# nagadomi/nunif

Hardware: NVIDIA H100
Metric: waifu2x_input_megapixels_per_sec (higher is better)
Workload: dtype f16

## Files before the change

nunif_b200/csrc/gemm.cu:

```cuda
#include "gemm.h"
#include "gemm_wgmma.cuh"
#include "tmap.h"
#include "../../include/nunif_b200.h"
#include <mutex>
#include <cstdlib>

namespace nb200 {

typedef CUresult (*EncodeTiledFn)(CUtensorMap*, CUtensorMapDataType, cuuint32_t, void*, const cuuint64_t*,
                                  const cuuint64_t*, const cuuint32_t*, const cuuint32_t*, CUtensorMapInterleave,
                                  CUtensorMapSwizzle, CUtensorMapL2promotion, CUtensorMapFloatOOBfill);

static EncodeTiledFn get_encode() {
    static EncodeTiledFn fn = nullptr;
    static std::once_flag once;
    std::call_once(once, [] {
        void* p = nullptr;
        cudaDriverEntryPointQueryResult q;
        if (cudaGetDriverEntryPoint("cuTensorMapEncodeTiled", &p, cudaEnableDefault, &q) == cudaSuccess &&
            q == cudaDriverEntryPointSuccess)
            fn = (EncodeTiledFn)p;
    });
    return fn;
}

int encode(CUtensorMap* m, const void* base, int rank, const cuuint64_t* dims, const cuuint64_t* strides_bytes,
                  const cuuint32_t* box, int swizzle_bytes) {
    EncodeTiledFn fn = get_encode();
    if (!fn) return fail("cuTensorMapEncodeTiled is not available (no CUDA driver?)");
    cuuint32_t estr[5] = {1, 1, 1, 1, 1};
    CUtensorMapSwizzle sw = swizzle_bytes == 128 ? CU_TENSOR_MAP_SWIZZLE_128B
                                                 : (swizzle_bytes == 64 ? CU_TENSOR_MAP_SWIZZLE_64B : CU_TENSOR_MAP_SWIZZLE_32B);
    CUresult r = fn(m, CU_TENSOR_MAP_DATA_TYPE_FLOAT16, (cuuint32_t)rank, const_cast<void*>(base), dims, strides_bytes, box,
                    estr, CU_TENSOR_MAP_INTERLEAVE_NONE, sw, CU_TENSOR_MAP_L2_PROMOTION_L2_256B,
                    CU_TENSOR_MAP_FLOAT_OOB_FILL_NONE);
    if (r != CUDA_SUCCESS) return fail("cuTensorMapEncodeTiled failed with CUresult " + std::to_string((int)r));
    return 0;
}

template <int BN, int BK, bool A2 = false>
static int launch_t(cudaStream_t st, const GemmMaps& maps, const GemmParams& p, int m_tiles, int n_tiles) {
    using Cfg = GemmCfg<BN, BK>;
    if (ensure_dyn_smem((const void*)gemm_conv_kernel<BN, BK, A2>, Cfg::SMEM_BYTES)) return 1;
    cudaLaunchConfig_t cfg = {};
    cfg.gridDim = dim3((unsigned)m_tiles * n_tiles); cfg.blockDim = dim3(GEMM_THREADS); cfg.dynamicSmemBytes = Cfg::SMEM_BYTES;
    cfg.stream = st;
    cudaLaunchAttribute at[1];
    at[0].id = cudaLaunchAttributeProgrammaticStreamSerialization;
    at[0].val.programmaticStreamSerializationAllowed = 1;
    cfg.attrs = at; cfg.numAttrs = 1;
    NB_CUDA(cudaLaunchKernelEx(&cfg, gemm_conv_kernel<BN, BK, A2>, maps, p));
    NB_LAUNCHED();
    return 0;
}

template <int BK>
static int launch_bn(int bn, cudaStream_t st, const GemmMaps& maps, const GemmParams& p, int m_tiles, int n_tiles) {
    if (p.k2) switch (bn) {
        case 64: return launch_t<64, BK, true>(st, maps, p, m_tiles, n_tiles);
        case 96: return launch_t<96, BK, true>(st, maps, p, m_tiles, n_tiles);
        default: return fail("second A operand: unsupported BLOCK_N");
    }
    switch (bn) {
        case 16: return launch_t<16, BK>(st, maps, p, m_tiles, n_tiles);
        case 32: return launch_t<32, BK>(st, maps, p, m_tiles, n_tiles);
        case 48: return launch_t<48, BK>(st, maps, p, m_tiles, n_tiles);
        case 64: return launch_t<64, BK>(st, maps, p, m_tiles, n_tiles);
        case 96: return launch_t<96, BK>(st, maps, p, m_tiles, n_tiles);
        case 128: return launch_t<128, BK>(st, maps, p, m_tiles, n_tiles);
    }
    return fail("unsupported BLOCK_N");
}

static int num_sms() { return device_sm_count(); }

std::atomic<int> g_tune_epoch{0};
int g_tune[16] = {0, 0, 0,  0, 0, 0,  0,
                   0, 0,  0, 0, 0, 0, 0, 0, 0};

static int encode_nhwc4(CUtensorMap* m, const __half* base, int C, int X, int Y, int B, long long sx, long long sy, long long sb,
                        int cw, int tw, int th) {
    cuuint64_t dims[4] = {(cuuint64_t)C, (cuuint64_t)X, (cuuint64_t)Y, (cuuint64_t)B};
    cuuint64_t strides[3] = {(cuuint64_t)sx * 2, (cuuint64_t)sy * 2, (cuuint64_t)sb * 2};
    cuuint32_t box[4] = {(cuuint32_t)cw, (cuuint32_t)tw, (cuuint32_t)th, 1};
    return encode(m, base, 4, dims, strides, box, cw * 2);
}

int conv_gemm(cudaStream_t st, const ConvGemm& g) {
    NB_CHECK(g.A && g.Wt && g.out, "null pointer");
    NB_CHECK(g.Ci % 8 == 0, "input channel stride must be a multiple of 8");
    NB_CHECK(g.N % 16 == 0, "N must be a multiple of 16 (pad the weights)");
    GemmParams p;
    memset(&p, 0, sizeof(p));
    int ktap;
    cuuint64_t dims[5], strides[4];
    cuuint32_t box[5];
    const cuuint64_t e = 2;
    const cuuint64_t rs = (g.a_row_stride ? (cuuint64_t)g.a_row_stride : (cuuint64_t)g.Wi * g.Ci) * e;
    const cuuint64_t is = (g.a_img_stride ? (cuuint64_t)g.a_img_stride * e : (cuuint64_t)g.Hi * rs);
    switch (g.kind) {
        case CG_LINEAR_FLAT: {
            const long long M = (long long)g.B * g.Hi * g.Wi;
// ... 121 lines not shown
            if (g.res) {
                const int oy = dy + g.res_cy, ox = dx + g.res_cx;
                NB_CHECK(oy + 2 * (p.Ho - 1) < g.res_H && ox + 2 * (p.Wo - 1) < g.res_W, "residual tensor too small");
                if (encode_nhwc4(&maps.r[q], g.res + ((size_t)oy * g.res_W + ox) * g.ldr, g.cout, p.Wo, p.Ho, p.B, 2LL * g.ldr,
                                 2LL * g.res_W * g.ldr, (long long)g.res_H * g.res_W * g.ldr, cw, p.TW, p.TH)) return 1;
            }
        }
        p.res_cx = p.res_cy = 0;
        if (a2) {
            const cuuint64_t px = (cuuint64_t)g.ld2 * e;
            cuuint64_t d2[5] = {(cuuint64_t)g.Cin2, 2, (cuuint64_t)p.Wo, 2, (cuuint64_t)p.B * p.Ho};
            cuuint64_t s2[4] = {px, 2 * px, (cuuint64_t)OW * px, 2 * (cuuint64_t)OW * px};
            cuuint32_t b2[5] = {(cuuint32_t)BK, 1, (cuuint32_t)p.TW, 1, (cuuint32_t)p.TH};
            if (encode(&maps.a2, g.A2, 5, d2, s2, b2, BK * 2)) return 1;
        }
    }
    const int m_tiles = p.tiles_x * p.tiles_y * p.B;
    const double Mrows = (double)p.B * p.Ho * p.Wo;
    const double in_px = g.kind == CG_DOWN2 ? 4.0 * Mrows : ((g.kind == CG_CONV3 || g.kind == CG_TCONV3) ? (double)p.B * g.Hi * g.Wi : Mrows);
    ProfScope ps(st, PC_GEMM, 2.0 * Mrows * (double)g.N * (double)K,
                 in_px * (g.kind == CG_LINEAR_FLAT ? g.Cin * g.a_planes : g.Cin) * 2.0 + (g.res ? Mrows * g.N * 2.0 : 0.0) +
                     4.0 * Mrows * g.Cin2 * (a2 ? 2.0 : 0.0) + (double)g.N * K * 2.0,
                 Mrows * (double)g.N * 2.0);
    if (rec_on()) {
        char line[512];
        snprintf(line, sizeof(line),
                 "gemm,%d,%d,%d,%d,%d,%d,%d,%d,%lld,%lld,%d,%lld,%d,%d,%d,%d,%d,%lld,%d,%d,%d,%d,%d,%d,%d,%d,%d,%d,%d,%d,%d,%d,%d,%d",
                 g.kind, g.pad, g.dil, g.B, g.Hi, g.Wi, g.Ci, g.Cin, g.a_row_stride, g.a_img_stride, g.a_planes, g.a_plane_stride,
                 g.N, g.act, g.ldo, g.out_mode, g.cout, g.split_stride, g.bias ? 1 : 0, g.res ? 1 : 0, g.ldr, g.res_H, g.res_W,
                 g.res_cy, g.res_cx, g.res_before_act, a2 ? 1 : 0, g.Cin2, g.ld2, g.res && (const void*)g.out == (const void*)g.res,
                 (const void*)g.out == (const void*)g.A, bn, BK, m_tiles * p.n_tiles);
        rec_append(line);
    }
    return BK == 64 ? launch_bn<64>(bn, st, maps, p, m_tiles, p.n_tiles) : launch_bn<32>(bn, st, maps, p, m_tiles, p.n_tiles);
}

}

using namespace nb200;

extern "C" int nb200_conv_gemm_f16(const void* A, int B, int Hi, int Wi, int Ci, int Cin, int kind, const void* Wt, int N,
                                   const float* bias, int act, void* out, int ldo, int out_mode, int cout,
                                   const void* res, int ldr, int res_H, int res_W, int res_cy, int res_cx,
                                   int res_before_act, void* stream) {
    ConvGemm g;
    g.A = (const __half*)A; g.B = B; g.Hi = Hi; g.Wi = Wi; g.Ci = Ci; g.Cin = Cin;
    g.kind = kind == 4 ? CG_CONV3 : kind;
    g.pad = kind == 4 ? 1 : 0;
    g.Wt = (const __half*)Wt; g.N = N; g.bias = bias; g.act = act; g.out = (__half*)out; g.ldo = ldo;
    g.out_mode = out_mode; g.cout = cout; g.res = (const __half*)res; g.ldr = ldr; g.res_H = res_H; g.res_W = res_W;
    g.res_cy = res_cy; g.res_cx = res_cx; g.res_before_act = res_before_act;
    return conv_gemm((cudaStream_t)stream, g);
}

extern "C" int nb200_conv_gemm_pixshuf_a2_f16(const void* A, int B, int Hi, int Wi, int Ci, const void* Wt, int N, const float* bias,
                                              int act, void* out, int ldo, int cout, const void* A2, int Cin2, int ld2, void* stream) {
    ConvGemm g;
    g.A = (const __half*)A; g.B = B; g.Hi = Hi; g.Wi = Wi; g.Ci = Ci; g.Cin = Ci; g.kind = CG_LINEAR_2D;
    g.Wt = (const __half*)Wt; g.N = N; g.bias = bias; g.act = act; g.out = (__half*)out; g.ldo = ldo;
    g.out_mode = OUT_PIXSHUF2; g.cout = cout; g.A2 = (const __half*)A2; g.Cin2 = Cin2; g.ld2 = ld2;
    NB_CHECK(g.A2, "null pointer");
    return conv_gemm((cudaStream_t)stream, g);
}

extern "C" int nb200_conv_gemm_ex_f16(const nb200_gemm_desc* d, const void* A, const void* Wt, const float* bias, void* out,
                                      const void* res, const void* A2, void* stream) {
    NB_CHECK(d, "null descriptor");
// ... 18 lines not shown
```

nunif_b200/csrc/gemm_wgmma.cuh:

```cuda
#pragma once
#include "common.cuh"
#include <cuda.h>

namespace nb200 {

enum : int { ACT_NONE = 0, ACT_LRELU01 = 1, ACT_GELU = 2, ACT_RELU = 3 };
enum : int { OUT_NHWC = 0, OUT_PIXSHUF2 = 1, OUT_SPLIT = 2 };

struct GemmParams {
    int B, Ho, Wo, TH, TW, tiles_x, tiles_y;
    int N;
    int taps, cpt;
    int8_t tap_dx[16], tap_dy[16], tap_dyi[16];
    int n_tiles;
    const float* bias;
    int act;
    int out_mode, cout;
    int has_res, res_cy, res_cx;
    int res_before_act;
    int k2;
};

struct GemmMaps {
    CUtensorMap a, b;
    CUtensorMap o[4];
    union {
        CUtensorMap r[4];
        CUtensorMap a2;
    };
};

__device__ __forceinline__ uint32_t smem_u32(const void* p) { return (uint32_t)__cvta_generic_to_shared(p); }

__device__ __forceinline__ void mbar_init(uint64_t* bar, uint32_t count) {
    asm volatile("mbarrier.init.shared::cta.b64 [%0], %1;" ::"r"(smem_u32(bar)), "r"(count));
}
__device__ __forceinline__ void mbar_expect_tx(uint64_t* bar, uint32_t bytes) {
    asm volatile("mbarrier.arrive.expect_tx.shared::cta.b64 _, [%0], %1;" ::"r"(smem_u32(bar)), "r"(bytes) : "memory");
}
__device__ __forceinline__ void mbar_arrive(uint64_t* bar) {
    asm volatile("mbarrier.arrive.shared::cta.b64 _, [%0];" ::"r"(smem_u32(bar)) : "memory");
}
static __device__ __noinline__ void mbar_timeout() {
    printf("nb200: mbarrier wait timed out (block %d,%d thread %d)\n", blockIdx.x, blockIdx.y, threadIdx.x);
    __trap();
}
__device__ __forceinline__ void mbar_wait(uint64_t* bar, uint32_t parity) {
    const uint32_t addr = smem_u32(bar);
    uint32_t done = 0;
#pragma unroll 1
    for (uint32_t it = 0; it < (1u << 18); ++it) {
        asm volatile(
            "{\n\t.reg .pred p;\n\t"
            "mbarrier.try_wait.parity.shared::cta.b64 p, [%1], %2, %3;\n\t"
            "selp.u32 %0, 1, 0, p;\n\t}"
            : "=r"(done) : "r"(addr), "r"(parity), "r"(20000u) : "memory");
        if (done) return;
    }
    mbar_timeout();
}
__device__ __forceinline__ void fence_barrier_init() {
    asm volatile("fence.mbarrier_init.release.cluster;" ::: "memory");
    asm volatile("fence.proxy.async.shared::cta;" ::: "memory");
}
__device__ __forceinline__ void tma_load_5d(const CUtensorMap* map, uint64_t* bar, void* dst, int c0, int c1, int c2, int c3, int c4) {
    asm volatile(
        "cp.async.bulk.tensor.5d.shared::cluster.global.tile.mbarrier::complete_tx::bytes [%0], [%1, {%3, %4, %5, %6, %7}], [%2];"
        ::"r"(smem_u32(dst)), "l"(map), "r"(smem_u32(bar)), "r"(c0), "r"(c1), "r"(c2), "r"(c3), "r"(c4) : "memory");
}
__device__ __forceinline__ void tma_load_2d(const CUtensorMap* map, uint64_t* bar, void* dst, int c0, int c1) {
    asm volatile(
        "cp.async.bulk.tensor.2d.shared::cluster.global.tile.mbarrier::complete_tx::bytes [%0], [%1, {%3, %4}], [%2];"
        ::"r"(smem_u32(dst)), "l"(map), "r"(smem_u32(bar)), "r"(c0), "r"(c1) : "memory");
}
__device__ __forceinline__ void tma_load_4d(const CUtensorMap* map, uint64_t* bar, void* dst, int c0, int c1, int c2, int c3) {
    asm volatile(
        "cp.async.bulk.tensor.4d.shared::cluster.global.tile.mbarrier::complete_tx::bytes [%0], [%1, {%3, %4, %5, %6}], [%2];"
        ::"r"(smem_u32(dst)), "l"(map), "r"(smem_u32(bar)), "r"(c0), "r"(c1), "r"(c2), "r"(c3) : "memory");
}
__device__ __forceinline__ void tma_store_4d(const CUtensorMap* map, const void* src, int c0, int c1, int c2, int c3) {
    asm volatile("cp.async.bulk.tensor.4d.global.shared::cta.tile.bulk_group [%0, {%2, %3, %4, %5}], [%1];"
                 ::"l"(map), "r"(smem_u32(src)), "r"(c0), "r"(c1), "r"(c2), "r"(c3) : "memory");
}
__device__ __forceinline__ void tma_store_2d(const CUtensorMap* map, const void* src, int c0, int c1) {
    asm volatile("cp.async.bulk.tensor.2d.global.shared::cta.tile.bulk_group [%0, {%2, %3}], [%1];"
                 ::"l"(map), "r"(smem_u32(src)), "r"(c0), "r"(c1) : "memory");
}
__device__ __forceinline__ void tma_store_commit() { asm volatile("cp.async.bulk.commit_group;" ::: "memory"); }
__device__ __forceinline__ void tma_store_wait_read() { asm volatile("cp.async.bulk.wait_group.read 0;" ::: "memory"); }
__device__ __forceinline__ void fence_async_smem() { asm volatile("fence.proxy.async.shared::cta;" ::: "memory"); }
__device__ __forceinline__ void consumer_bar_sync() { asm volatile("bar.sync 1, 256;" ::: "memory"); }
__device__ __forceinline__ void tma_prefetch_desc(const CUtensorMap* map) {
    asm volatile("prefetch.tensormap [%0];" ::"l"(map) : "memory");
// ... 80 lines not shown
    asm("ex2.approx.ftz.f32 %0, %1;" : "=f"(e) : "f"(fmaf(-q, a, -1.0f)));
    return fmaxf(x, 0.f) - a * e;
}

template <int K>
__device__ __forceinline__ void apply_act(float (&v)[K], int act) {
    switch (act) {
        case ACT_LRELU01:
#pragma unroll
            for (int j = 0; j < K; ++j) v[j] = v[j] > 0.f ? v[j] : 0.1f * v[j];
            break;
        case ACT_GELU:
#pragma unroll
            for (int j = 0; j < K; ++j) v[j] = gelu_erf(v[j]);
            break;
        case ACT_RELU:
#pragma unroll
            for (int j = 0; j < K; ++j) v[j] = fmaxf(v[j], 0.f);
            break;
        default: break;
    }
}

constexpr int GEMM_CONSUMER_THREADS = 256;
constexpr int GEMM_THREADS = GEMM_CONSUMER_THREADS + 32;

template <int BLOCK_N, int BK>
struct GemmCfg {
    static_assert(BLOCK_N % 16 == 0 && BLOCK_N <= 128, "BLOCK_N: 16..128 (the fp32 accumulators live in registers)");
    static constexpr int SWIZZLE = BK * 2;
    static constexpr int A_BYTES = 128 * BK * 2;
    static constexpr int B_BYTES = BLOCK_N * BK * 2;
    static constexpr int STAGE_BYTES = A_BYTES + ((B_BYTES + 1023) / 1024) * 1024;
    static constexpr int STAGES = (98304 / STAGE_BYTES) < 2 ? 2 : ((98304 / STAGE_BYTES) > 6 ? 6 : (98304 / STAGE_BYTES));
    static constexpr int CW = (BLOCK_N % 64 == 0) ? 64 : ((BLOCK_N % 32 == 0) ? 32 : 16);
    static constexpr int NCH = BLOCK_N / CW;
    static constexpr int CH_BYTES = 128 * CW * 2;
    static_assert(NCH * CH_BYTES <= STAGES * STAGE_BYTES, "epilogue staging must fit in the (drained) pipeline stages");
    static constexpr int SMEM_BYTES = STAGES * STAGE_BYTES + 1024  + 256 ;
};

template <int CW>
__device__ __forceinline__ uint32_t stage_off(int r, int j) {
    if (CW == 64) return (uint32_t)(r * 128 + ((j ^ (r & 7)) << 4));
    if (CW == 32) return (uint32_t)(r * 64 + ((j ^ ((r >> 1) & 3)) << 4));
    return (uint32_t)(r * 32 + ((j ^ ((r >> 2) & 1)) << 4));
}

template <int ROWS>
__device__ __forceinline__ uint32_t sw64_off(int r, int col) {
    return (uint32_t)((col >> 5) * (ROWS * 64)) + stage_off<32>(r, (col & 31) >> 3) + (uint32_t)((col & 7) * 2);
}

template <int BLOCK_N, int BK, bool A2 = false>
__global__ void __launch_bounds__(GEMM_THREADS, 2) gemm_conv_kernel(const __grid_constant__ GemmMaps maps,
                                                                    const __grid_constant__ GemmParams p) {
    using Cfg = GemmCfg<BLOCK_N, BK>;
    constexpr int STAGES = Cfg::STAGES;
    constexpr int CW = Cfg::CW;
    extern __shared__ uint8_t smem_dyn[];
    uint8_t* smem = reinterpret_cast<uint8_t*>((reinterpret_cast<uintptr_t>(smem_dyn) + 1023) & ~(uintptr_t)1023);
    uint64_t* full_bar = reinterpret_cast<uint64_t*>(smem + STAGES * Cfg::STAGE_BYTES);
    uint64_t* empty_bar = full_bar + STAGES;
    uint64_t* res_bar = empty_bar + STAGES;

    const int warp = threadIdx.x >> 5;
    const int n_tile = blockIdx.x % p.n_tiles;
    const int tile = blockIdx.x / p.n_tiles;
    const int tx_i = tile % p.tiles_x;
    const int ty_i = (tile / p.tiles_x) % p.tiles_y;
    const int b = tile / (p.tiles_x * p.tiles_y);
    const int x0 = tx_i * p.TW, y0 = ty_i * p.TH;
    const int n0 = n_tile * BLOCK_N;
    const int k_iters = p.taps * p.cpt + (A2 ? p.k2 : 0);

    if (threadIdx.x == GEMM_CONSUMER_THREADS) {
        tma_prefetch_desc(&maps.a);
        tma_prefetch_desc(&maps.b);
        tma_prefetch_desc(&maps.o[0]);
        for (int s = 0; s < STAGES; ++s) {
            mbar_init(&full_bar[s], 1);
            mbar_init(&empty_bar[s], 2);
        }
        mbar_init(res_bar, 1);
        fence_barrier_init();
    }
    __syncthreads();

    if (warp == GEMM_CONSUMER_THREADS / 32) {
        if (elect_one()) {
            asm volatile("griddepcontrol.wait;" ::: "memory");
            for (int it = 0; it < k_iters; ++it) {
                const int s = it % STAGES;
                const uint32_t ph = (it / STAGES) & 1;
                mbar_wait(&empty_bar[s], ph ^ 1);
                const int tap = it / p.cpt, ch = it - tap * p.cpt;
                uint8_t* sa = smem + s * Cfg::STAGE_BYTES;
                uint8_t* sb = sa + Cfg::A_BYTES;
                mbar_expect_tx(&full_bar[s], Cfg::A_BYTES + Cfg::B_BYTES);
                if (A2 && tap >= p.taps) {
                    const int q = n0 / p.cout;
                    tma_load_5d(&maps.a2, &full_bar[s], sa, (it - p.taps * p.cpt) * BK, q & 1, x0, q >> 1, b * p.Ho + y0);
                } else {
                    tma_load_5d(&maps.a, &full_bar[s], sa, ch * BK, x0 + p.tap_dx[tap], p.tap_dyi[tap], y0 + p.tap_dy[tap], b);
                }
                tma_load_2d(&maps.b, &full_bar[s], sb, it * BK, n0);
            }
        }
        return;
    }

    const int wg = threadIdx.x >> 7;
    const int t = threadIdx.x & 127;
    float acc[BLOCK_N / 2];
#pragma unroll
    for (int j = 0; j < BLOCK_N / 2; ++j) acc[j] = 0.f;
    for (int it = 0; it < k_iters; ++it) {
        const int s = it % STAGES;
        mbar_wait(&full_bar[s], (it / STAGES) & 1);
        const uint32_t sa = smem_u32(smem + s * Cfg::STAGE_BYTES) + wg * 64 * Cfg::SWIZZLE;
        const uint32_t sb = smem_u32(smem + s * Cfg::STAGE_BYTES) + Cfg::A_BYTES;
        wgmma_fence();
#pragma unroll
        for (int k = 0; k < BK / 16; ++k)
            wgmma_f16<BLOCK_N>(acc, make_kmajor_desc<Cfg::SWIZZLE>(sa + k * 32), make_kmajor_desc<Cfg::SWIZZLE>(sb + k * 32), 1u);
        wgmma_commit();
        wgmma_wait<1>();
        if (it > 0 && t == 0) mbar_arrive(&empty_bar[(it - 1) % STAGES]);
    }
    wgmma_wait<0>();
    wgmma_fence_operands(acc);
    if (threadIdx.x == 0) NB_PDL_TRIGGER();
    consumer_bar_sync();
    uint8_t* stg = smem;
    const bool leader = threadIdx.x == 0;
    if (p.has_res) {
        if (leader) {
            mbar_expect_tx(res_bar, Cfg::NCH * Cfg::CH_BYTES);
#pragma unroll 1
            for (int c = 0; c < Cfg::NCH; ++c) {
                const int n = n0 + c * CW;
                const int g = p.out_mode != OUT_NHWC ? n / p.cout : 0;
                const int co = p.out_mode != OUT_NHWC ? n - g * p.cout : n;
                tma_load_4d(&maps.r[g], res_bar, stg + c * Cfg::CH_BYTES, co, x0 + p.res_cx, y0 + p.res_cy, b);
            }
        }
        mbar_wait(res_bar, 0);
    }
    const int act = p.act;
    const bool has_res = p.has_res != 0, res_first = p.res_before_act != 0;
    const int row0 = wg * 64 + (t >> 5) * 16 + ((t & 31) >> 2);
    const int cq = 2 * (t & 3);
#pragma unroll
    for (int j = 0; j < BLOCK_N / 8; ++j) {
        const int col = 8 * j + cq;
        const int c = (8 * j) / CW;
        float2 bq = make_float2(0.f, 0.f);
        if (p.bias) bq = __ldg(reinterpret_cast<const float2*>(p.bias + n0 + col));
        float v[4] = {acc[4 * j] + bq.x, acc[4 * j + 1] + bq.y, acc[4 * j + 2] + bq.x, acc[4 * j + 3] + bq.y};
        __half2* s0 = reinterpret_cast<__half2*>(stg + c * Cfg::CH_BYTES + stage_off<CW>(row0, (8 * j % CW) / 8) + 2 * cq);
        __half2* s1 = reinterpret_cast<__half2*>(stg + c * Cfg::CH_BYTES + stage_off<CW>(row0 + 8, (8 * j % CW) / 8) + 2 * cq);
        if (has_res) {
            const float2 r0 = __half22float2(*s0), r1 = __half22float2(*s1);
            const float rv[4] = {r0.x, r0.y, r1.x, r1.y};
            if (res_first) {
#pragma unroll
                for (int q = 0; q < 4; ++q) v[q] += rv[q];
                apply_act(v, act);
            } else {
                apply_act(v, act);
#pragma unroll
                for (int q = 0; q < 4; ++q) v[q] += rv[q];
            }
        } else {
            apply_act(v, act);
        }
        *s0 = __floats2half2_rn(v[0], v[1]);
        *s1 = __floats2half2_rn(v[2], v[3]);
    }
    fence_async_smem();
    consumer_bar_sync();
    if (leader) {
#pragma unroll 1
        for (int c = 0; c < Cfg::NCH; ++c) {
            const int n = n0 + c * CW;
            const int g = p.out_mode != OUT_NHWC ? n / p.cout : 0;
            const int co = p.out_mode != OUT_NHWC ? n - g * p.cout : n;
            tma_store_4d(&maps.o[g], stg + c * Cfg::CH_BYTES, co, x0, y0, b);
        }
        tma_store_commit();
        tma_store_wait_read();
    }
}

}
```

nunif_b200/csrc/swin_block.cu:

```cuda
#include "gemm_wgmma.cuh"
#include "swin_kernels.h"
#include "tmap.h"

namespace nb200 {

constexpr int FM_ROWS = 128, FM_STAGES = 5, FM_THREADS = GEMM_CONSUMER_THREADS + 128;
constexpr int FM_PRODUCER_REGS = 40, FM_CONSUMER_REGS = 232;

template <int C>
struct FmCfg {
    static constexpr int KB = C / 32;
    static constexpr int TILE = FM_ROWS * C * 2;
    static constexpr int STAGE = 128 * C;
    static constexpr int SMEM = 2 * TILE + FM_STAGES * STAGE + (2 * FM_STAGES + KB + 1) * 8 + 1024;
};

struct FmMaps {
    CUtensorMap x, att, wp, w1, w2, y, wy;
};

template <int K>
__device__ __forceinline__ float (&half96(float (&acc)[K], int h))[48] { return *reinterpret_cast<float(*)[48]>(&acc[48 * h]); }

__device__ __forceinline__ void fm_wait(uint64_t* bar, uint32_t parity) {
    const uint32_t addr = smem_u32(bar);
    uint32_t done = 0;
#pragma unroll 1
    for (uint32_t it = 0; it < (1u << 18) && !done; ++it)
        asm volatile(
            "{\n\t.reg .pred p;\n\t"
            "mbarrier.try_wait.parity.shared::cta.b64 p, [%1], %2, %3;\n\t"
            "selp.u32 %0, 1, 0, p;\n\t}"
            : "=r"(done) : "r"(addr), "r"(parity), "r"(20000u) : "memory");
    if (!done) __trap();
}

__device__ __forceinline__ void wgmma_wait_n(int n) {
    if (n == 0) wgmma_wait<0>();
    else wgmma_wait<1>();
}

template <int C, bool PROJ, int CS>
__global__ void __launch_bounds__(FM_THREADS, 1) swin_mlp_fused_kernel(const __grid_constant__ FmMaps maps, const float* __restrict__ bp,
                                                                     const float* __restrict__ b1, const float* __restrict__ b2,
                                                                     const float* __restrict__ by) {
    using Cfg = FmCfg<C>;
    static_assert(CS % 16 == 0 && 2 * C * CS <= Cfg::STAGE && CS * 256 <= Cfg::TILE, "Wy must fit a ring stage, y the att tile");
    constexpr int KB = Cfg::KB, NP = (KB + 1) / 2, NH = 2 * C / 64, NHALF = C / 96;
    extern __shared__ uint8_t smem_dyn[];
    uint8_t* smem = reinterpret_cast<uint8_t*>((reinterpret_cast<uintptr_t>(smem_dyn) + 1023) & ~(uintptr_t)1023);
    uint8_t* sx = smem;
    uint8_t* satt = smem + Cfg::TILE;
    uint8_t* ring = smem + 2 * Cfg::TILE;
    uint64_t* full = reinterpret_cast<uint64_t*>(ring + FM_STAGES * Cfg::STAGE);
    uint64_t* empty = full + FM_STAGES;
    uint64_t* abar = empty + FM_STAGES;
    uint64_t* xbar = abar + KB;
    const int tid = threadIdx.x, warp = tid >> 5;
    const int row_base = blockIdx.x * FM_ROWS;
    if (tid == GEMM_CONSUMER_THREADS) {
        tma_prefetch_desc(&maps.x);
        tma_prefetch_desc(&maps.w1);
        tma_prefetch_desc(&maps.w2);
        if (CS) tma_prefetch_desc(&maps.wy);
        if (PROJ) {
            tma_prefetch_desc(&maps.att);
            tma_prefetch_desc(&maps.wp);
        }
        for (int s = 0; s < FM_STAGES; ++s) {
            mbar_init(&full[s], 1);
            mbar_init(&empty[s], 2);
        }
        for (int kb = 0; kb < KB; ++kb) mbar_init(&abar[kb], 1);
        mbar_init(xbar, 1);
        fence_barrier_init();
    }
    __syncthreads();

    if (warp >= GEMM_CONSUMER_THREADS / 32) {
        asm volatile("setmaxnreg.dec.sync.aligned.u32 %0;" ::"n"(FM_PRODUCER_REGS));
        if (warp == GEMM_CONSUMER_THREADS / 32 && elect_one()) {
            bool acts = false;
            auto load_acts = [&]() {
                asm volatile("griddepcontrol.wait;" ::: "memory");
                if (PROJ)
                    for (int kb = 0; kb < KB; ++kb) {
                        mbar_expect_tx(&abar[kb], FM_ROWS * 64);
                        tma_load_2d(&maps.att, &abar[kb], satt + kb * (FM_ROWS * 64), kb * 32, row_base);
                    }
                mbar_expect_tx(xbar, Cfg::TILE);
                for (int kb = 0; kb < KB; ++kb) tma_load_2d(&maps.x, xbar, sx + kb * (FM_ROWS * 64), kb * 32, row_base);
                acts = true;
            };
            int it = 0;
            auto push = [&](const CUtensorMap* m, int k0, int n0, int rows, int nbox) {
                if (it == FM_STAGES) load_acts();
                const int s = it % FM_STAGES;
                fm_wait(&empty[s], ((it / FM_STAGES) & 1) ^ 1);
                mbar_expect_tx(&full[s], nbox * rows * 64);
                for (int b = 0; b < nbox; ++b) tma_load_2d(m, &full[s], ring + s * Cfg::STAGE + b * rows * 64, k0 + 32 * b, n0);
                ++it;
            };
            if (PROJ)
                for (int j = 0; j < NP; ++j) push(&maps.wp, 64 * j, 0, C, min(2, KB - 2 * j));
            push(&maps.w1, 0, 0, 64, KB);
            for (int hc = 0; hc < NH; ++hc) {
                if (hc + 1 < NH) push(&maps.w1, 0, (hc + 1) * 64, 64, KB);
                push(&maps.w2, hc * 64, 0, C, 2);
            }
            if (CS) push(&maps.wy, 0, 0, CS, KB);
            if (!acts) load_acts();
        }
        return;
    }

    asm volatile("setmaxnreg.inc.sync.aligned.u32 %0;" ::"n"(FM_CONSUMER_REGS));
    const int wg = tid >> 7, t = tid & 127;
    const int row0 = wg * 64 + (t >> 5) * 16 + ((t & 31) >> 2);
    const int cq = 2 * (t & 3);
    const uint32_t x_base = smem_u32(sx) + wg * 64 * 64, att_base = smem_u32(satt) + wg * 64 * 64;
    int it = 0, pending = 0;
    auto take = [&]() -> uint32_t {
        const int s = it % FM_STAGES;
        fm_wait(&full[s], (it / FM_STAGES) & 1);
        return smem_u32(ring + s * Cfg::STAGE);
    };
    auto commit = [&]() {
        wgmma_commit();
        ++it;
        ++pending;
    };
    auto retire = [&](int n) {
        wgmma_wait_n(n);
#pragma unroll
        for (int k = 0; k < FM_STAGES; ++k)
            if (k < pending - n && t == 0) mbar_arrive(&empty[(it - pending + k) % FM_STAGES]);
        pending = min(pending, n);
    };

    if (PROJ) {
        float acc[C / 2];
#pragma unroll
        for (int j = 0; j < C / 2; ++j) acc[j] = 0.f;
        wgmma_fence_operands(acc);
#pragma unroll
        for (int j = 0; j < NP; ++j) {
            const uint32_t bb = take();
#pragma unroll
            for (int kb = 2 * j; kb < 2 * j + 2 && kb < KB; ++kb) fm_wait(&abar[kb], 0);
            wgmma_fence();
#pragma unroll
            for (int kb = 2 * j; kb < 2 * j + 2 && kb < KB; ++kb) {
                const uint32_t a = att_base + kb * (FM_ROWS * 64), b = bb + (kb - 2 * j) * (C * 64);
#pragma unroll
                for (int s = 0; s < 2; ++s)
#pragma unroll
                    for (int h = 0; h < NHALF; ++h)
                        wgmma_f16<96>(half96(acc, h), make_kmajor_desc<64>(a + 32 * s), make_kmajor_desc<64>(b + h * 96 * 64 + 32 * s), 1u);
            }
            commit();
            retire(1);
        }
        retire(0);
        wgmma_fence_operands(acc);
        fm_wait(xbar, 0);
#pragma unroll
        for (int j = 0; j < C / 8; ++j) {
            const int col = 8 * j + cq;
            const float2 bq = __ldg(reinterpret_cast<const float2*>(bp + col));
#pragma unroll
            for (int i = 0; i < 2; ++i) {
                __half2* p = reinterpret_cast<__half2*>(sx + sw64_off<FM_ROWS>(row0 + 8 * i, col));
                const float2 xv = __half22float2(*p);
                *p = __floats2half2_rn(xv.x + (acc[4 * j + 2 * i] + bq.x), xv.y + (acc[4 * j + 2 * i + 1] + bq.y));
            }
        }
        fence_async_smem();
        asm volatile("bar.sync %0, 128;" ::"r"(2 + wg) : "memory");
    } else {
        fm_wait(xbar, 0);
    }

    float oacc[C / 2];
#pragma unroll
    for (int j = 0; j < C / 2; ++j) oacc[j] = 0.f;
    wgmma_fence_operands(oacc);
    float hacc[2][32];
    uint32_t af[4][4];
    auto fc1 = [&](float (&h)[32]) {
#pragma unroll
        for (int j = 0; j < 32; ++j) h[j] = 0.f;
        wgmma_fence_operands(h);
        const uint32_t bb = take();
        wgmma_fence();
#pragma unroll
        for (int kb = 0; kb < KB; ++kb) {
            const uint32_t a = x_base + kb * (FM_ROWS * 64), b = bb + kb * (64 * 64);
            wgmma_f16<64>(h, make_kmajor_desc<64>(a), make_kmajor_desc<64>(b), 1u);
            wgmma_f16<64>(h, make_kmajor_desc<64>(a + 32), make_kmajor_desc<64>(b + 32), 1u);
        }
        commit();
    };
    fc1(hacc[0]);
#pragma unroll
    for (int hc = 0; hc < NH; ++hc) {
        const int buf = hc & 1;
        if (hc + 1 < NH) fc1(hacc[buf ^ 1]);
        retire(hc + 1 < NH ? 1 : 0);
        wgmma_fence_operands(hacc[buf]);
#pragma unroll
        for (int kk = 0; kk < 4; ++kk)
#pragma unroll
            for (int q = 0; q < 4; ++q) {
// ... 157 lines not shown
```

Before: 70.96.

## Make conv GEMM kernel persistent with dedicated epilogue staging and async stores

The implicit-GEMM conv kernel becomes persistent. The grid is capped at the number of resident CTAs and each CTA loops over tiles, so the TMA producer can prefetch the next tile's operands while the consumers run the epilogue. Shared memory is re-planned under a fixed limit so the epilogue staging buffer is separate from the pipeline stages, and output TMA stores are committed asynchronously and waited on before the buffer is reused. The in-place case (output aliasing an input) still launches one CTA per tile to avoid read/write hazards. Barrier waits switch to a bounded-spin variant that traps on timeout, and an A/B benchmarking script is added.

```diff
diff --git a/nunif_b200/csrc/gemm.cu b/nunif_b200/csrc/gemm.cu
--- a/nunif_b200/csrc/gemm.cu
+++ b/nunif_b200/csrc/gemm.cu
@@ -39,11 +39,17 @@
 }
 
 template <int BN, int BK, bool A2 = false>
-static int launch_t(cudaStream_t st, const GemmMaps& maps, const GemmParams& p, int m_tiles, int n_tiles) {
+static int launch_t(cudaStream_t st, const GemmMaps& maps, const GemmParams& p, bool one_per_tile) {
     using Cfg = GemmCfg<BN, BK>;
-    if (ensure_dyn_smem((const void*)gemm_conv_kernel<BN, BK, A2>, Cfg::SMEM_BYTES)) return 1;
+    const void* fn = (const void*)gemm_conv_kernel<BN, BK, A2>;
+    if (ensure_dyn_smem(fn, Cfg::SMEM_BYTES)) return 1;
+    static int ctas_per_sm = 0;
+    if (!ctas_per_sm) NB_CUDA(cudaOccupancyMaxActiveBlocksPerMultiprocessor(&ctas_per_sm, fn, GEMM_THREADS, Cfg::SMEM_BYTES));
+    NB_CHECK(ctas_per_sm > 0, "gemm_conv_kernel does not fit an SM");
+    const long long resident = (long long)ctas_per_sm * device_sm_count();
+    const int grid = one_per_tile || p.tiles <= resident ? p.tiles : (int)resident;
     cudaLaunchConfig_t cfg = {};
-    cfg.gridDim = dim3((unsigned)m_tiles * n_tiles); cfg.blockDim = dim3(GEMM_THREADS); cfg.dynamicSmemBytes = Cfg::SMEM_BYTES;
+    cfg.gridDim = dim3((unsigned)grid); cfg.blockDim = dim3(GEMM_THREADS); cfg.dynamicSmemBytes = Cfg::SMEM_BYTES;
     cfg.stream = st;
     cudaLaunchAttribute at[1];
     at[0].id = cudaLaunchAttributeProgrammaticStreamSerialization;
@@ -55,19 +61,19 @@
 }
 
 template <int BK>
-static int launch_bn(int bn, cudaStream_t st, const GemmMaps& maps, const GemmParams& p, int m_tiles, int n_tiles) {
+static int launch_bn(int bn, cudaStream_t st, const GemmMaps& maps, const GemmParams& p, bool one_per_tile) {
     if (p.k2) switch (bn) {
-        case 64: return launch_t<64, BK, true>(st, maps, p, m_tiles, n_tiles);
-        case 96: return launch_t<96, BK, true>(st, maps, p, m_tiles, n_tiles);
+        case 64: return launch_t<64, BK, true>(st, maps, p, one_per_tile);
+        case 96: return launch_t<96, BK, true>(st, maps, p, one_per_tile);
         default: return fail("second A operand: unsupported BLOCK_N");
     }
     switch (bn) {
-        case 16: return launch_t<16, BK>(st, maps, p, m_tiles, n_tiles);
-        case 32: return launch_t<32, BK>(st, maps, p, m_tiles, n_tiles);
-        case 48: return launch_t<48, BK>(st, maps, p, m_tiles, n_tiles);
-        case 64: return launch_t<64, BK>(st, maps, p, m_tiles, n_tiles);
-        case 96: return launch_t<96, BK>(st, maps, p, m_tiles, n_tiles);
-        case 128: return launch_t<128, BK>(st, maps, p, m_tiles, n_tiles);
+        case 16: return launch_t<16, BK>(st, maps, p, one_per_tile);
+        case 32: return launch_t<32, BK>(st, maps, p, one_per_tile);
+        case 48: return launch_t<48, BK>(st, maps, p, one_per_tile);
+        case 64: return launch_t<64, BK>(st, maps, p, one_per_tile);
+        case 96: return launch_t<96, BK>(st, maps, p, one_per_tile);
+        case 128: return launch_t<128, BK>(st, maps, p, one_per_tile);
     }
     return fail("unsupported BLOCK_N");
 }
@@ -255,7 +261,9 @@
                  (const void*)g.out == (const void*)g.A, bn, BK, m_tiles * p.n_tiles);
         rec_append(line);
     }
-    return BK == 64 ? launch_bn<64>(bn, st, maps, p, m_tiles, p.n_tiles) : launch_bn<32>(bn, st, maps, p, m_tiles, p.n_tiles);
+    p.tiles = m_tiles * p.n_tiles;
+    const bool one_per_tile = (const void*)g.out == (const void*)g.A || (a2 && (const void*)g.out == (const void*)g.A2);
+    return BK == 64 ? launch_bn<64>(bn, st, maps, p, one_per_tile) : launch_bn<32>(bn, st, maps, p, one_per_tile);
 }
 
 }
diff --git a/nunif_b200/csrc/gemm_wgmma.cuh b/nunif_b200/csrc/gemm_wgmma.cuh
--- a/nunif_b200/csrc/gemm_wgmma.cuh
+++ b/nunif_b200/csrc/gemm_wgmma.cuh
@@ -13,6 +13,7 @@
     int taps, cpt;
     int8_t tap_dx[16], tap_dy[16], tap_dyi[16];
     int n_tiles;
+    int tiles;
     const float* bias;
     int act;
     int out_mode, cout;
@@ -59,6 +60,18 @@
     }
     mbar_timeout();
 }
+__device__ __forceinline__ void mbar_wait_trap(uint64_t* bar, uint32_t parity) {
+    const uint32_t addr = smem_u32(bar);
+    uint32_t done = 0;
+#pragma unroll 1
+    for (uint32_t it = 0; it < (1u << 18) && !done; ++it)
+        asm volatile(
+            "{\n\t.reg .pred p;\n\t"
+            "mbarrier.try_wait.parity.shared::cta.b64 p, [%1], %2, %3;\n\t"
+            "selp.u32 %0, 1, 0, p;\n\t}"
+            : "=r"(done) : "r"(addr), "r"(parity), "r"(20000u) : "memory");
+    if (!done) __trap();
+}
 __device__ __forceinline__ void fence_barrier_init() {
     asm volatile("fence.mbarrier_init.release.cluster;" ::: "memory");
     asm volatile("fence.proxy.async.shared::cta;" ::: "memory");
@@ -205,12 +218,19 @@
     static constexpr int A_BYTES = 128 * BK * 2;
     static constexpr int B_BYTES = BLOCK_N * BK * 2;
     static constexpr int STAGE_BYTES = A_BYTES + ((B_BYTES + 1023) / 1024) * 1024;
-    static constexpr int STAGES = (98304 / STAGE_BYTES) < 2 ? 2 : ((98304 / STAGE_BYTES) > 6 ? 6 : (98304 / STAGE_BYTES));
     static constexpr int CW = (BLOCK_N % 64 == 0) ? 64 : ((BLOCK_N % 32 == 0) ? 32 : 16);
     static constexpr int NCH = BLOCK_N / CW;
     static constexpr int CH_BYTES = 128 * CW * 2;
-    static_assert(NCH * CH_BYTES <= STAGES * STAGE_BYTES, "epilogue staging must fit in the (drained) pipeline stages");
-    static constexpr int SMEM_BYTES = STAGES * STAGE_BYTES + 1024  + 256 ;
+    static constexpr int SMEM_LIMIT = 113 * 1024;
+    static constexpr int SLACK = 1024 , BAR_BYTES = 256;
+    static constexpr int SCH = (SMEM_LIMIT - SLACK - BAR_BYTES - NCH * CH_BYTES) / STAGE_BYTES >= 3 ? NCH : 1;
+    static constexpr bool BARS_IN_SLACK = SCH < NCH;
+    static constexpr int STG_BYTES = SCH * CH_BYTES;
+    static constexpr int SMEM_FIXED = STG_BYTES + SLACK + (BARS_IN_SLACK ? 0 : BAR_BYTES);
+    static constexpr int STAGES_FIT = (SMEM_LIMIT - SMEM_FIXED) / STAGE_BYTES;
+    static constexpr int STAGES = STAGES_FIT > 6 ? 6 : STAGES_FIT;
+    static_assert(STAGES >= 3 && NCH % SCH == 0, "at least three pipeline stages");
+    static constexpr int SMEM_BYTES = STAGES * STAGE_BYTES + SMEM_FIXED;
 };
 
 template <int CW>
@@ -223,6 +243,13 @@
 template <int ROWS>
 __device__ __forceinline__ uint32_t sw64_off(int r, int col) {
     return (uint32_t)((col >> 5) * (ROWS * 64)) + stage_off<32>(r, (col & 31) >> 3) + (uint32_t)((col & 7) * 2);
+}
+
+struct GemmTile { int x0, y0, b, n0; };
+__device__ __forceinline__ GemmTile gemm_tile(const GemmParams& p, int tile, int block_n) {
+    const int m = tile / p.n_tiles;
+    const int tx = m % p.tiles_x, ty = (m / p.tiles_x) % p.tiles_y;
+    return {tx * p.TW, ty * p.TH, m / (p.tiles_x * p.tiles_y), (tile - m * p.n_tiles) * block_n};
 }
 
 template <int BLOCK_N, int BK, bool A2 = false>
@@ -233,18 +260,13 @@
     constexpr int CW = Cfg::CW;
     extern __shared__ uint8_t smem_dyn[];
     uint8_t* smem = reinterpret_cast<uint8_t*>((reinterpret_cast<uintptr_t>(smem_dyn) + 1023) & ~(uintptr_t)1023);
-    uint64_t* full_bar = reinterpret_cast<uint64_t*>(smem + STAGES * Cfg::STAGE_BYTES);
+    uint8_t* stg = smem + STAGES * Cfg::STAGE_BYTES;
+    uint64_t* full_bar = reinterpret_cast<uint64_t*>(Cfg::BARS_IN_SLACK && smem - smem_dyn >= Cfg::BAR_BYTES ? smem_dyn
+                                                                                                          : stg + Cfg::STG_BYTES);
     uint64_t* empty_bar = full_bar + STAGES;
     uint64_t* res_bar = empty_bar + STAGES;
 
     const int warp = threadIdx.x >> 5;
-    const int n_tile = blockIdx.x % p.n_tiles;
-    const int tile = blockIdx.x / p.n_tiles;
-    const int tx_i = tile % p.tiles_x;
-    const int ty_i = (tile / p.tiles_x) % p.tiles_y;
-    const int b = tile / (p.tiles_x * p.tiles_y);
-    const int x0 = tx_i * p.TW, y0 = ty_i * p.TH;
-    const int n0 = n_tile * BLOCK_N;
     const int k_iters = p.taps * p.cpt + (A2 ? p.k2 : 0);
 
     if (threadIdx.x == GEMM_CONSUMER_THREADS) {
@@ -263,21 +285,24 @@
     if (warp == GEMM_CONSUMER_THREADS / 32) {
         if (elect_one()) {
             asm volatile("griddepcontrol.wait;" ::: "memory");
-            for (int it = 0; it < k_iters; ++it) {
-                const int s = it % STAGES;
-                const uint32_t ph = (it / STAGES) & 1;
-                mbar_wait(&empty_bar[s], ph ^ 1);
-                const int tap = it / p.cpt, ch = it - tap * p.cpt;
-                uint8_t* sa = smem + s * Cfg::STAGE_BYTES;
-                uint8_t* sb = sa + Cfg::A_BYTES;
-                mbar_expect_tx(&full_bar[s], Cfg::A_BYTES + Cfg::B_BYTES);
-                if (A2 && tap >= p.taps) {
-                    const int q = n0 / p.cout;
-                    tma_load_5d(&maps.a2, &full_bar[s], sa, (it - p.taps * p.cpt) * BK, q & 1, x0, q >> 1, b * p.Ho + y0);
-                } else {
-                    tma_load_5d(&maps.a, &full_bar[s], sa, ch * BK, x0 + p.tap_dx[tap], p.tap_dyi[tap], y0 + p.tap_dy[tap], b);
+            int it = 0;
+            for (int tile = blockIdx.x; tile < p.tiles; tile += gridDim.x) {
+                const GemmTile tl = gemm_tile(p, tile, BLOCK_N);
+                for (int k = 0; k < k_iters; ++k, ++it) {
+                    const int s = it % STAGES;
+                    mbar_wait_trap(&empty_bar[s], ((it / STAGES) & 1) ^ 1);
+                    const int tap = k / p.cpt, ch = k - tap * p.cpt;
+                    uint8_t* sa = smem + s * Cfg::STAGE_BYTES;
+                    uint8_t* sb = sa + Cfg::A_BYTES;
+                    mbar_expect_tx(&full_bar[s], Cfg::A_BYTES + Cfg::B_BYTES);
+                    if (A2 && tap >= p.taps) {
+                        const int q = tl.n0 / p.cout;
+                        tma_load_5d(&maps.a2, &full_bar[s], sa, (k - p.taps * p.cpt) * BK, q & 1, tl.x0, q >> 1, tl.b * p.Ho + tl.y0);
+                    } else {
+                        tma_load_5d(&maps.a, &full_bar[s], sa, ch * BK, tl.x0 + p.tap_dx[tap], p.tap_dyi[tap], tl.y0 + p.tap_dy[tap], tl.b);
+                    }
+                    tma_load_2d(&maps.b, &full_bar[s], sb, k * BK, tl.n0);
                 }
-                tma_load_2d(&maps.b, &full_bar[s], sb, it * BK, n0);
             }
         }
         return;
@@ -285,85 +310,95 @@
 
     const int wg = threadIdx.x >> 7;
     const int t = threadIdx.x & 127;
-    float acc[BLOCK_N / 2];
-#pragma unroll
-    for (int j = 0; j < BLOCK_N / 2; ++j) acc[j] = 0.f;
-    for (int it = 0; it < k_iters; ++it) {
-        const int s = it % STAGES;
-        mbar_wait(&full_bar[s], (it / STAGES) & 1);
-        const uint32_t sa = smem_u32(smem + s * Cfg::STAGE_BYTES) + wg * 64 * Cfg::SWIZZLE;
-        const uint32_t sb = smem_u32(smem + s * Cfg::STAGE_BYTES) + Cfg::A_BYTES;
-        wgmma_fence();
-#pragma unroll
-        for (int k = 0; k < BK / 16; ++k)
-            wgmma_f16<BLOCK_N>(acc, make_kmajor_desc<Cfg::SWIZZLE>(sa + k * 32), make_kmajor_desc<Cfg::SWIZZLE>(sb + k * 32), 1u);
-        wgmma_commit();
-        wgmma_wait<1>();
-        if (it > 0 && t == 0) mbar_arrive(&empty_bar[(it - 1) % STAGES]);
-    }
-    wgmma_wait<0>();
-    wgmma_fence_operands(acc);
-    if (threadIdx.x == 0) NB_PDL_TRIGGER();
-    consumer_bar_sync();
-    uint8_t* stg = smem;
     const bool leader = threadIdx.x == 0;
-    if (p.has_res) {
-        if (leader) {
-            mbar_expect_tx(res_bar, Cfg::NCH * Cfg::CH_BYTES);
-#pragma unroll 1
-            for (int c = 0; c < Cfg::NCH; ++c) {
-                const int n = n0 + c * CW;
-                const int g = p.out_mode != OUT_NHWC ? n / p.cout : 0;
-                const int co = p.out_mode != OUT_NHWC ? n - g * p.cout : n;
-                tma_load_4d(&maps.r[g], res_bar, stg + c * Cfg::CH_BYTES, co, x0 + p.res_cx, y0 + p.res_cy, b);
-            }
-        }
-        mbar_wait(res_bar, 0);
-    }
     const int act = p.act;
     const bool has_res = p.has_res != 0, res_first = p.res_before_act != 0;
     const int row0 = wg * 64 + (t >> 5) * 16 + ((t & 31) >> 2);
     const int cq = 2 * (t & 3);
-#pragma unroll
-    for (int j = 0; j < BLOCK_N / 8; ++j) {
-        const int col = 8 * j + cq;
-        const int c = (8 * j) / CW;
-        float2 bq = make_float2(0.f, 0.f);
-        if (p.bias) bq = __ldg(reinterpret_cast<const float2*>(p.bias + n0 + col));
-        float v[4] = {acc[4 * j] + bq.x, acc[4 * j + 1] + bq.y, acc[4 * j + 2] + bq.x, acc[4 * j + 3] + bq.y};
-        __half2* s0 = reinterpret_cast<__half2*>(stg + c * Cfg::CH_BYTES + stage_off<CW>(row0, (8 * j % CW) / 8) + 2 * cq);
-        __half2* s1 = reinterpret_cast<__half2*>(stg + c * Cfg::CH_BYTES + stage_off<CW>(row0 + 8, (8 * j % CW) / 8) + 2 * cq);
-        if (has_res) {
-            const float2 r0 = __half22float2(*s0), r1 = __half22float2(*s1);
-            const float rv[4] = {r0.x, r0.y, r1.x, r1.y};
-            if (res_first) {
-#pragma unroll
-                for (int q = 0; q < 4; ++q) v[q] += rv[q];
-                apply_act(v, act);
-            } else {
-                apply_act(v, act);
-#pragma unroll
-                for (int q = 0; q < 4; ++q) v[q] += rv[q];
+    int it = 0;
+    uint32_t res_phase = 0;
+    for (int tile = blockIdx.x; tile < p.tiles; tile += gridDim.x) {
+        const GemmTile tl = gemm_tile(p, tile, BLOCK_N);
+        float acc[BLOCK_N / 2];
+#pragma unroll
+        for (int j = 0; j < BLOCK_N / 2; ++j) acc[j] = 0.f;
+        for (int k = 0; k < k_iters; ++k, ++it) {
+            const int s = it % STAGES;
+            mbar_wait_trap(&full_bar[s], (it / STAGES) & 1);
+            const uint32_t sa = smem_u32(smem + s * Cfg::STAGE_BYTES) + wg * 64 * Cfg::SWIZZLE;
+            const uint32_t sb = smem_u32(smem + s * Cfg::STAGE_BYTES) + Cfg::A_BYTES;
+            wgmma_fence();
+#pragma unroll
+            for (int kk = 0; kk < BK / 16; ++kk)
+                wgmma_f16<BLOCK_N>(acc, make_kmajor_desc<Cfg::SWIZZLE>(sa + kk * 32), make_kmajor_desc<Cfg::SWIZZLE>(sb + kk * 32), 1u);
+            wgmma_commit();
+            wgmma_wait<1>();
+            if (k > 0 && t == 0) mbar_arrive(&empty_bar[(it - 1) % STAGES]);
+        }
+        wgmma_wait<0>();
+        wgmma_fence_operands(acc);
+        if (t == 0) mbar_arrive(&empty_bar[(it - 1) % STAGES]);
+        if (leader && tile + (int)gridDim.x >= p.tiles) NB_PDL_TRIGGER();
+#pragma unroll
+        for (int r = 0; r < Cfg::NCH / Cfg::SCH; ++r) {
+            if (leader) tma_store_wait_read();
+            consumer_bar_sync();
+            if (has_res) {
+                if (leader) {
+                    mbar_expect_tx(res_bar, Cfg::STG_BYTES);
+#pragma unroll 1
+                    for (int c = 0; c < Cfg::SCH; ++c) {
+                        const int n = tl.n0 + (r * Cfg::SCH + c) * CW;
+                        const int g = p.out_mode != OUT_NHWC ? n / p.cout : 0;
+                        const int co = p.out_mode != OUT_NHWC ? n - g * p.cout : n;
+                        tma_load_4d(&maps.r[g], res_bar, stg + c * Cfg::CH_BYTES, co, tl.x0 + p.res_cx, tl.y0 + p.res_cy, tl.b);
+                    }
+                }
+                mbar_wait_trap(res_bar, res_phase);
+                res_phase ^= 1;
             }
-        } else {
-            apply_act(v, act);
+#pragma unroll
+            for (int j = r * Cfg::SCH * CW / 8; j < (r + 1) * Cfg::SCH * CW / 8; ++j) {
+                const int col = 8 * j + cq;
+                const int c = (8 * j) / CW - r * Cfg::SCH;
+                float2 bq = make_float2(0.f, 0.f);
+                if (p.bias) bq = __ldg(reinterpret_cast<const float2*>(p.bias + tl.n0 + col));
+                float v[4] = {acc[4 * j] + bq.x, acc[4 * j + 1] + bq.y, acc[4 * j + 2] + bq.x, acc[4 * j + 3] + bq.y};
+                __half2* s0 = reinterpret_cast<__half2*>(stg + c * Cfg::CH_BYTES + stage_off<CW>(row0, (8 * j % CW) / 8) + 2 * cq);
+                __half2* s1 = reinterpret_cast<__half2*>(stg + c * Cfg::CH_BYTES + stage_off<CW>(row0 + 8, (8 * j % CW) / 8) + 2 * cq);
+                if (has_res) {
+                    const float2 r0 = __half22float2(*s0), r1 = __half22float2(*s1);
+                    const float rv[4] = {r0.x, r0.y, r1.x, r1.y};
+                    if (res_first) {
+#pragma unroll
+                        for (int q = 0; q < 4; ++q) v[q] += rv[q];
+                        apply_act(v, act);
+                    } else {
+                        apply_act(v, act);
+#pragma unroll
+                        for (int q = 0; q < 4; ++q) v[q] += rv[q];
+                    }
+                } else {
+                    apply_act(v, act);
+                }
+                *s0 = __floats2half2_rn(v[0], v[1]);
+                *s1 = __floats2half2_rn(v[2], v[3]);
+            }
+            fence_async_smem();
+            consumer_bar_sync();
+            if (leader) {
+#pragma unroll 1
+                for (int c = 0; c < Cfg::SCH; ++c) {
+                    const int n = tl.n0 + (r * Cfg::SCH + c) * CW;
+                    const int g = p.out_mode != OUT_NHWC ? n / p.cout : 0;
+                    const int co = p.out_mode != OUT_NHWC ? n - g * p.cout : n;
+                    tma_store_4d(&maps.o[g], stg + c * Cfg::CH_BYTES, co, tl.x0, tl.y0, tl.b);
+                }
+                tma_store_commit();
+            }
         }
-        *s0 = __floats2half2_rn(v[0], v[1]);
-        *s1 = __floats2half2_rn(v[2], v[3]);
     }
-    fence_async_smem();
-    consumer_bar_sync();
-    if (leader) {
-#pragma unroll 1
-        for (int c = 0; c < Cfg::NCH; ++c) {
-            const int n = n0 + c * CW;
-            const int g = p.out_mode != OUT_NHWC ? n / p.cout : 0;
-            const int co = p.out_mode != OUT_NHWC ? n - g * p.cout : n;
-            tma_store_4d(&maps.o[g], stg + c * Cfg::CH_BYTES, co, x0, y0, b);
-        }
-        tma_store_commit();
-        tma_store_wait_read();
-    }
-}
-
-}
+    if (leader) tma_store_wait_read();
+}
+
+}
diff --git a/nunif_b200/csrc/swin_block.cu b/nunif_b200/csrc/swin_block.cu
--- a/nunif_b200/csrc/swin_block.cu
+++ b/nunif_b200/csrc/swin_block.cu
@@ -21,19 +21,6 @@
 
 template <int K>
 __device__ __forceinline__ float (&half96(float (&acc)[K], int h))[48] { return *reinterpret_cast<float(*)[48]>(&acc[48 * h]); }
-
-__device__ __forceinline__ void fm_wait(uint64_t* bar, uint32_t parity) {
-    const uint32_t addr = smem_u32(bar);
-    uint32_t done = 0;
-#pragma unroll 1
-    for (uint32_t it = 0; it < (1u << 18) && !done; ++it)
-        asm volatile(
-            "{\n\t.reg .pred p;\n\t"
-            "mbarrier.try_wait.parity.shared::cta.b64 p, [%1], %2, %3;\n\t"
-            "selp.u32 %0, 1, 0, p;\n\t}"
-            : "=r"(done) : "r"(addr), "r"(parity), "r"(20000u) : "memory");
-    if (!done) __trap();
-}
 
 __device__ __forceinline__ void wgmma_wait_n(int n) {
     if (n == 0) wgmma_wait<0>();
@@ -96,7 +83,7 @@
             auto push = [&](const CUtensorMap* m, int k0, int n0, int rows, int nbox) {
                 if (it == FM_STAGES) load_acts();
                 const int s = it % FM_STAGES;
-                fm_wait(&empty[s], ((it / FM_STAGES) & 1) ^ 1);
+                mbar_wait_trap(&empty[s], ((it / FM_STAGES) & 1) ^ 1);
                 mbar_expect_tx(&full[s], nbox * rows * 64);
                 for (int b = 0; b < nbox; ++b) tma_load_2d(m, &full[s], ring + s * Cfg::STAGE + b * rows * 64, k0 + 32 * b, n0);
                 ++it;
@@ -122,7 +109,7 @@
     int it = 0, pending = 0;
     auto take = [&]() -> uint32_t {
         const int s = it % FM_STAGES;
-        fm_wait(&full[s], (it / FM_STAGES) & 1);
+        mbar_wait_trap(&full[s], (it / FM_STAGES) & 1);
         return smem_u32(ring + s * Cfg::STAGE);
     };
     auto commit = [&]() {
@@ -147,7 +134,7 @@
         for (int j = 0; j < NP; ++j) {
             const uint32_t bb = take();
 #pragma unroll
-            for (int kb = 2 * j; kb < 2 * j + 2 && kb < KB; ++kb) fm_wait(&abar[kb], 0);
+            for (int kb = 2 * j; kb < 2 * j + 2 && kb < KB; ++kb) mbar_wait_trap(&abar[kb], 0);
             wgmma_fence();
 #pragma unroll
             for (int kb = 2 * j; kb < 2 * j + 2 && kb < KB; ++kb) {
@@ -163,7 +150,7 @@
         }
         retire(0);
         wgmma_fence_operands(acc);
-        fm_wait(xbar, 0);
+        mbar_wait_trap(xbar, 0);
 #pragma unroll
         for (int j = 0; j < C / 8; ++j) {
             const int col = 8 * j + cq;
@@ -178,7 +165,7 @@
         fence_async_smem();
         asm volatile("bar.sync %0, 128;" ::"r"(2 + wg) : "memory");
     } else {
-        fm_wait(xbar, 0);
+        mbar_wait_trap(xbar, 0);
     }
 
     float oacc[C / 2];
diff --git a/profiles/ab_gemm.py b/profiles/ab_gemm.py
--- /dev/null
+++ b/profiles/ab_gemm.py
@@ -0,0 +1,171 @@
+#!/usr/bin/env python
+import argparse
+import ctypes
+import json
+import os
+import statistics
+import subprocess
+import sys
+
+ROOT = os.path.dirname(os.path.dirname(os.path.abspath(__file__)))
+sys.path.insert(0, ROOT)
+
+REPS = 7
+WINDOW_MS = 60.0
+FLAT, LIN2D, CONV3, DOWN2 = 0, 1, 2, 3
+ACT_NONE, ACT_LRELU, ACT_GELU = 0, 1, 2
+OUT_NHWC, OUT_PIXSHUF2 = 0, 1
+
+
+def conv3(name, B, H, cin, cout):
+    return dict(name=name, kind=CONV3, B=B, Hi=H, Wi=H, Ci=cin, Cin=cin, N=cout, act=ACT_LRELU, ldo=cout)
+
+
+CUNET = [(254, 32, 64), (126, 64, 128), (124, 128, 64), (244, 64, 64), (478, 32, 64), (238, 64, 128), (236, 128, 128),
+         (117, 128, 256), (115, 256, 128), (226, 128, 64), (224, 64, 64), (444, 64, 64)]
+
+SHAPES = [
+    dict(name="swin4x conv2 3x3 64->96 @242", kind=CONV3, B=16, Hi=242, Wi=242, Ci=64, Cin=64, N=96, act=ACT_LRELU, ldo=96),
+    dict(name="swin4x down1 2x2s2 96->192 @240", kind=DOWN2, B=16, Hi=240, Wi=240, Ci=96, Cin=96, N=192, ldo=192),
+    dict(name="swin4x down2 2x2s2 192->192 @120", kind=DOWN2, B=16, Hi=120, Wi=120, Ci=192, Cin=192, N=192, ldo=192),
+    dict(name="swin4x up2 192->4x192 pixshuf +res @60", kind=LIN2D, B=16, Hi=60, Wi=60, Ci=192, Cin=192, N=768, ldo=192,
+         out_mode=OUT_PIXSHUF2, cout=192, res=(120, 192)),
+    dict(name="swin4x up1 (192|96)->4x192 pixshuf A2 @120", kind=LIN2D, B=16, Hi=120, Wi=120, Ci=192, Cin=192, N=768, ldo=192,
+         out_mode=OUT_PIXSHUF2, cout=192, a2=96),
+] + [conv3(f"upcunet conv3 {ci}->{co} @{h}", 16, h, ci, co) for h, ci, co in CUNET] + [
+    dict(name="zoed_n fc1 1024->4096 gelu", kind=FLAT, B=1, Hi=1, Wi=2 * 1057, Ci=1024, Cin=1024, N=4096, act=ACT_GELU, ldo=4096),
+    dict(name="zoed_n qkv 1024->3072", kind=FLAT, B=1, Hi=1, Wi=2 * 1057, Ci=1024, Cin=1024, N=3072, ldo=3072),
+]
+
+
+def load(path):
+    from nunif_b200 import _lib
+    lib = ctypes.CDLL(os.path.abspath(path))
+    for name in ("nb200_last_error", "nb200_check_device", "nb200_conv_gemm_ex_f16"):
+        res, args = _lib.SIGNATURES[name]
+        getattr(lib, name).restype, getattr(lib, name).argtypes = res, args
+    return lib
+
+
+def check(lib, rc):
+    if rc != 0:
+        raise RuntimeError(lib.nb200_last_error().decode("utf-8", "replace"))
+
+
+def geometry(s):
+    if s["kind"] == CONV3:
+        return s["Hi"] - 2, s["Wi"] - 2, 9 * s["Cin"]
+    if s["kind"] == DOWN2:
+        return s["Hi"] // 2, s["Wi"] // 2, 4 * s["Cin"]
+    return s["Hi"], s["Wi"], s["Cin"] + s.get("a2", 0)
+
+
+def inputs(s, dev):
+    import torch
+    from nunif_b200 import _lib
+    g = torch.Generator(device="cpu").manual_seed(sum(map(ord, s["name"])))
+    Ho, Wo, K = geometry(s)
+    B, N = s["B"], s["N"]
+    t = {"A": torch.randn(B, s["Hi"], s["Wi"], s["Ci"], generator=g).half().to(dev),
+         "W": (torch.randn(N, K, generator=g) / K ** 0.5).half().to(dev),
+         "bias": (0.1 * torch.randn(N, generator=g)).to(dev)}
+    d = dict(kind=s["kind"], pad=0, dil=1, B=B, Hi=s["Hi"], Wi=s["Wi"], Ci=s["Ci"], Cin=s["Cin"], a_planes=1, N=N,
+             act=s.get("act", ACT_NONE), ldo=s["ldo"], out_mode=s.get("out_mode", OUT_NHWC), cout=s.get("cout", 0))
+    if d["out_mode"] == OUT_PIXSHUF2:
+        t["out_shape"] = (B, 2 * Ho, 2 * Wo, s["cout"])
+    else:
+        t["out_shape"] = (B, Ho, Wo, N)
+    if "res" in s:
+        rh, rc = s["res"]
+        t["res"] = torch.randn(B, rh, rh, rc, generator=g).half().to(dev)
+        d.update(ldr=rc, res_H=rh, res_W=rh)
+    if "a2" in s:
+        c2 = s["a2"]
+        t["A2"] = torch.randn(B, 2 * Ho, 2 * Wo, c2, generator=g).half().to(dev)
+        d.update(Cin2=c2, ld2=c2)
+    t["desc"] = _lib.GemmDesc(**d)
+    t["flop"] = 2.0 * B * Ho * Wo * N * K
+    return t
+
+
+def call(lib, t, out):
+    import torch
+    p = lambda k: ctypes.c_void_p(t[k].data_ptr()) if k in t else None
+    check(lib, lib.nb200_conv_gemm_ex_f16(ctypes.byref(t["desc"]), p("A"), p("W"), p("bias"), ctypes.c_void_p(out.data_ptr()),
+                                          p("res"), p("A2"), ctypes.c_void_p(torch.cuda.current_stream().cuda_stream)))
+
+
+def window_ms(lib, t, out, n):
+    import torch
+    e0, e1 = torch.cuda.Event(enable_timing=True), torch.cuda.Event(enable_timing=True)
+    e0.record()
+    for _ in range(n):
+        call(lib, t, out)
+    e1.record()
+    e1.synchronize()
+    return e0.elapsed_time(e1) / n
+
+
+def device_info(index):
+    q = subprocess.run(["nvidia-smi", "-i", str(index), "--query-gpu=name,power.limit,clocks.max.sm", "--format=csv,noheader"],
+                       capture_output=True, text=True)
+    return q.stdout.strip()
+
+
+def main():
+    ap = argparse.ArgumentParser(description=__doc__, formatter_class=argparse.RawDescriptionHelpFormatter)
+    ap.add_argument("--base", required=True, help="the build to compare against (libnunif_b200.so)")
+    ap.add_argument("--new", default=os.path.join(ROOT, "nunif_b200", "libnunif_b200.so"), help="default: this tree's build")
+    ap.add_argument("--out", default=None, help="also write the JSON result here")
+    args = ap.parse_args()
+    import torch
+    from bench import ClockSampler
+    dev = torch.device("cuda:0")
+    torch.cuda.init()
+    torch.zeros(1, device=dev)
+    paths = {"base": args.base, "new": args.new}
+    libs = {k: load(v) for k, v in paths.items()}
+    for lib in libs.values():
+        check(lib, lib.nb200_check_device(0))
+    info = {"device": torch.cuda.get_device_name(dev), "nvidia_smi": device_info(0), "paths": paths}
+    print(f"# {info['device']} | name, power limit, max SM clock: {info['nvidia_smi']}")
+
+    rows = []
+    with torch.inference_mode(), ClockSampler(0) as clocks:
+        for s in SHAPES:
+            t = inputs(s, dev)
+            outs = {k: torch.full(t["out_shape"], 7.0, dtype=torch.half, device=dev) for k in libs}
+            for k, lib in libs.items():
+                for _ in range(3):
+                    call(lib, t, outs[k])
+            torch.cuda.synchronize()
+            equal = torch.equal(outs["base"], outs["new"])
+            diff = float((outs["base"].float() - outs["new"].float()).abs().max())
+            est = max(window_ms(libs[k], t, outs[k], 2) for k in libs)
+            n = max(3, int(WINDOW_MS / max(est, 1e-3)))
+            ms = {k: [] for k in libs}
+            for r in range(REPS):
+                for k in (("base", "new") if r % 2 == 0 else ("new", "base")):
+                    ms[k].append(window_ms(libs[k], t, outs[k], n))
+            row = {"shape": s["name"], "calls_per_window": n, "equal": equal, "max_abs_diff": diff}
+            for k in libs:
+                row[k] = {"median_ms": statistics.median(ms[k]), "min_ms": min(ms[k]), "max_ms": max(ms[k])}
+            row["new_over_base"] = row["new"]["median_ms"] / row["base"]["median_ms"]
+            row["new_tflops"] = t["flop"] / row["new"]["median_ms"] / 1e9
+            rows.append(row)
+            b, nw = row["base"], row["new"]
+            print(f"{s['name']:45s} base {b['median_ms']:.4f} ms [{b['min_ms']:.4f}, {b['max_ms']:.4f}]  "
+                  f"new {nw['median_ms']:.4f} ms [{nw['min_ms']:.4f}, {nw['max_ms']:.4f}]  new/base {row['new_over_base']:.3f}  "
+                  f"{row['new_tflops']:.0f} TFLOP/s  outputs {'identical' if equal else f'DIFFER (max |d| {diff:g})'}", flush=True)
+            del t, outs
+    result = {"info": info, "clocks": clocks.summary(), "shapes": rows, "all_equal": all(r["equal"] for r in rows)}
+    print(json.dumps(result))
+    if args.out:
+        os.makedirs(os.path.dirname(os.path.abspath(args.out)), exist_ok=True)
+        with open(args.out, "w") as fh:
+            json.dump(result, fh, indent=1)
+    return 0 if result["all_equal"] else 1
+
+
+if __name__ == "__main__":
+    sys.exit(main())
```

Result: faster. 72.04 (median of 6 runs) (+1.5%).
